# QihanW/eals_cpp

Measured on NVIDIA B200. Metric: eals_nnzK_updates_per_s, higher is better.
Workload: dtype f64

## Files before the change

### eals_cpp_b200/csrc/cd_block.cuh

```cuda
#pragma once

#include "cd_sweep.cuh"
#include "common.cuh"

namespace eals {

constexpr int kBlkThreads = 256;
constexpr int kBlkWarps = kBlkThreads / 32;
constexpr int kPartLen = 208;
constexpr int kMaxSlab = 256;

__device__ __forceinline__ uint32_t tile_chunk_off(int r, int c) { return (uint32_t)(r * 128 + (((c ^ r) & 7) << 4)); }
__device__ __forceinline__ double tile_elem(const unsigned char* tile, int r, int e) {
  return *reinterpret_cast<const double*>(tile + tile_chunk_off(r, e >> 1) + ((e & 1) << 3));
}

__device__ __forceinline__ void cp_async16(void* smem_dst, const void* gmem_src, int src_bytes) {
  const uint32_t d = (uint32_t)__cvta_generic_to_shared(smem_dst);
  asm volatile("cp.async.cg.shared.global [%0], [%1], 16, %2;\n" ::"r"(d), "l"(gmem_src), "r"(src_bytes) : "memory");
}
__device__ __forceinline__ void cp_async_commit() { asm volatile("cp.async.commit_group;\n" ::: "memory"); }
template <int N>
__device__ __forceinline__ void cp_async_wait() { asm volatile("cp.async.wait_group %0;\n" ::"n"(N) : "memory"); }

__device__ __forceinline__ void stage_tile_rows(unsigned char* tile, const double* const* rowp_s, int n, int n_pad,
                                                int fb, int tid, int nthreads) {
  const int c = tid & 7;
  const uint32_t col_bytes = (uint32_t)(fb * (kFB * 8) + c * 16);
  for (int r = tid >> 3; r < n_pad; r += nthreads >> 3) {
    const bool live = r < n;
    const unsigned char* src = reinterpret_cast<const unsigned char*>(rowp_s[live ? r : 0]) + col_bytes;
    cp_async16(tile + (uint32_t)(r * 128) + (uint32_t)(((c ^ r) & 7) << 4), src, live ? 16 : 0);
  }
}

__device__ __forceinline__ void stage_two_tiles(unsigned char* tile_prev, unsigned char* tile, const double* const* rowp_s,
                                                int n, int n_pad, int fb, bool do_prev, bool do_cur, int tid, int nthreads) {
  const int c = tid & 7;
  const uint32_t col_bytes = (uint32_t)(fb * (kFB * 8) + c * 16);
  for (int r = tid >> 3; r < n_pad; r += nthreads >> 3) {
    const bool live = r < n;
    const unsigned char* src = reinterpret_cast<const unsigned char*>(rowp_s[live ? r : 0]) + col_bytes;
    const uint32_t dst = (uint32_t)(r * 128) + (uint32_t)(((c ^ r) & 7) << 4);
    if (do_prev) cp_async16(tile_prev + dst, src - kFB * 8, live ? 16 : 0);
    if (do_cur) cp_async16(tile + dst, src, live ? 16 : 0);
  }
}

__device__ __forceinline__ void dmma_884(double& c0, double& c1, double a, double b) {
  asm volatile("mma.sync.aligned.m8n8k4.row.col.f64.f64.f64.f64 {%0,%1}, {%2}, {%3}, {%0,%1};\n"
               : "+d"(c0), "+d"(c1)
               : "d"(a), "d"(b));
}

__device__ __forceinline__ void load_tile_row(const unsigned char* tile, int r, double (&y)[16]) {
#pragma unroll
  for (int c = 0; c < 8; c++) {
    const double2 d = *reinterpret_cast<const double2*>(tile + tile_chunk_off(r, c));
    y[2 * c] = d.x;
    y[2 * c + 1] = d.y;
  }
}

constexpr int kSBlk = 16 * 17;
constexpr int kGsStride = 17;
constexpr int kGsLen = 16 * kGsStride;
__host__ __device__ constexpr int s_tri(int bi, int bj) { return bi * (bi + 1) / 2 + bj; }

template <int LD, int MAXM>
struct WarpBlockSmem {
  static constexpr bool kSInSmem = LD <= 128;
  static constexpr int kNB = LD / 16;
  static constexpr int kRows = 32 * MAXM;
  static constexpr size_t kS = kSInSmem ? (size_t)s_tri(kNB, 0) * kSBlk * 8 : 0;
  static constexpr size_t kTile = (size_t)kRows * 128;
  static constexpr size_t kBytesPerWarp = kTile + (size_t)kRows * 8 + (size_t)LD * 8 + (kGsLen + 16 + 16) * 8;
  static constexpr int kMaxWarps = MAXM == 1 ? 16 : (MAXM == 2 ? 12 : (MAXM == 3 ? 9 : 7));
};

__device__ __forceinline__ void gram_rhs_fragments(const unsigned char* tile, const double* c_s, const double* z_s,
                                                   int r0, int r1, double (&frag)[10]) {
  const int lane = lane_id();
  const int rr = lane & 3, e0 = lane >> 2;
  const uint32_t off_lo = (uint32_t)(rr * 128 + ((e0 & 1) << 3));
  for (int j0 = r0; j0 < r1; j0 += 4) {
    const int r = j0 + rr;
    const uint32_t sw = (uint32_t)(r & 7);
    const unsigned char* rowp = tile + (size_t)j0 * 128 + off_lo;
    const double a0 = *reinterpret_cast<const double*>(rowp + ((((uint32_t)(e0 >> 1)) ^ sw) << 4));
    const double a1 = *reinterpret_cast<const double*>(rowp + ((((uint32_t)(4 + (e0 >> 1))) ^ sw) << 4));
    const double cj = c_s[r];
    const double zj = e0 == 0 ? z_s[r] : 0.0;
    const double b0 = cj * a0, b1 = cj * a1;
    dmma_884(frag[0], frag[1], a0, b0);
    dmma_884(frag[2], frag[3], a1, b0);
    dmma_884(frag[4], frag[5], a1, b1);
    dmma_884(frag[6], frag[7], a0, zj);
    dmma_884(frag[8], frag[9], a1, zj);
  }
}

__device__ __forceinline__ void gram_rhs_fragments_reg(const unsigned char* tile, double c_lane, double z_lane,
                                                       int r0, int r1, double (&frag)[10]) {
  const int lane = lane_id();
  const int rr = lane & 3, e0 = lane >> 2;
  const uint32_t off_lo = (uint32_t)(rr * 128 + ((e0 & 1) << 3));
  for (int j0 = r0; j0 < r1; j0 += 4) {
    const int r = j0 + rr;
    const uint32_t sw = (uint32_t)(r & 7);
    const unsigned char* rowp = tile + (size_t)j0 * 128 + off_lo;
    const double a0 = *reinterpret_cast<const double*>(rowp + ((((uint32_t)(e0 >> 1)) ^ sw) << 4));
    const double a1 = *reinterpret_cast<const double*>(rowp + ((((uint32_t)(4 + (e0 >> 1))) ^ sw) << 4));
    const double cj = __shfl_sync(kFullMask, c_lane, (j0 - r0) + rr);
    const double zq = __shfl_sync(kFullMask, z_lane, (j0 - r0) + rr);
    const double zj = e0 == 0 ? zq : 0.0;
    const double b0 = cj * a0, b1 = cj * a1;
    dmma_884(frag[0], frag[1], a0, b0);
    dmma_884(frag[2], frag[3], a1, b0);
    dmma_884(frag[4], frag[5], a1, b1);
    dmma_884(frag[6], frag[7], a0, zj);
    dmma_884(frag[8], frag[9], a1, zj);
  }
}

template <int LD, int MAXM, bool USER>
__global__ void __launch_bounds__(WarpBlockSmem<LD, MAXM>::kMaxWarps * 32, 1)
cd_warp_block_kernel(CdSide a, const int32_t* __restrict__ order, int first, int count) {
  extern __shared__ __align__(128) unsigned char smem[];
  using Sm = WarpBlockSmem<LD, MAXM>;
  const int warp = threadIdx.x >> 5, lane = lane_id();
// ... 213 lines not shown
      const double hff = Gs[f * kGsStride + f];
      const double xf = x_s[f0 + f];
      double numer = Pt[f] - g * tsum + xf * hff;
      const double rden = 1.0 / (hff + a.reg);
#pragma unroll
      for (int s = 0; s < 16; s++) {
        const double d = numer * rden - xf;
        const double ds = __shfl_sync(kFullMask, d, s);
        if (f > s) numer -= ds * h[s];
      }
      const double xnew = numer * rden;
      if (lane < 16) {
        const bool livef = f0 + f < K;
        if (livef) x_s[f0 + f] = xnew;
        delta_s[f] = livef ? xnew - xf : 0.0;
      }
      __syncwarp();

      double d[16];
#pragma unroll
      for (int e = 0; e < 16; e++) d[e] = delta_s[e];
#pragma unroll
      for (int m = 0; m < MAXM; m++) {
        const int j = m * 32 + lane;
        if (j < n) {
          double y[16];
          load_tile_row(tile, j, y);
          double a0 = pr[m], a1 = 0.0, a2 = 0.0, a3 = 0.0;
#pragma unroll
          for (int e = 0; e < 16; e += 4) {
            a0 += d[e] * y[e];
            a1 += d[e + 1] * y[e + 1];
            a2 += d[e + 2] * y[e + 2];
            a3 += d[e + 3] * y[e + 3];
          }
          pr[m] = (a0 + a1) + (a2 + a3);
        }
      }
      __syncwarp();
      if (fb + 1 < nblocks) {
        stage_tile_rows(tile, rowp_s, n, n_pad, fb + 1, lane, 32);
        cp_async_commit();
      }
    }
    for (int k = lane; k < K; k += 32) store_row_value(a, (size_t)grow * LD + k, x_s[k]);
    if (a.pc_out.n) {
#pragma unroll
      for (int m = 0; m < MAXM; m++) {
        const int j = m * 32 + lane;
        if (j < n) pc_emit(a, p0 + j, gpos[m], pr[m]);
      }
    }
    for (int st = stages_in_loop; st < 4; st++) fetch_next(st, slot + stride);
    __syncwarp();
  }
  peers_release(a);
}

template <int LD, int TW, int MW>
struct RowBlockSmem {
  static constexpr int kT = TW * 32;
  static constexpr int kRows = kT * MW;
  static constexpr size_t kTile = (size_t)kRows * 128;
  static constexpr size_t kIdx = (size_t)kRows * 8;
  static constexpr size_t kCZ = (size_t)kRows * 16;
  static constexpr size_t kX = (size_t)LD * 8;
  static constexpr size_t kSlots = (size_t)TW * kPartLen * 8;
  static constexpr size_t kSmall = (kGsLen + 16 + 16 + 16 + 16 * 16) * 8;
  static constexpr size_t kBytes = kTile + kIdx + kCZ + kX + kSlots + kSmall;
};

template <int LD, int TW, int MW, bool USER>
__global__ void __launch_bounds__(TW * 32, 16 / TW)
cd_row_block_kernel(CdSide a, const int32_t* __restrict__ order, int first) {
  extern __shared__ __align__(128) unsigned char smem[];
  using Sm = RowBlockSmem<LD, TW, MW>;
  constexpr int kT = TW * 32;
  constexpr int kParts = kT / 16;
  static_assert(kPartLen + 16 <= kT || TW < 8, "reduction threads");
  unsigned char* tile = smem;
  const double** rowp_s = reinterpret_cast<const double**>(smem + Sm::kTile);
  double* c_s = reinterpret_cast<double*>(smem + Sm::kTile + Sm::kIdx);
  double* z_s = c_s + Sm::kRows;
  double* x_s = z_s + Sm::kRows;
  double* slots = x_s + LD;
  double* Gs = slots + TW * kPartLen;
  double* Pt = Gs + kGsLen;
  double* Tt = Pt + 16;
  double* delta_s = Tt + 16;
  double* tpart = delta_s + 16;

  const int tid = threadIdx.x, lane = lane_id(), warp = tid >> 5;
  const int row = order[first + blockIdx.x];
  const int64_t p0 = a.ptr[row];
  const int n = (int)(a.ptr[row + 1] - p0);
  const int n_pad = (n + 3) & ~3;
  const int grow = a.row_base + row;
  double* xrow = a.X + (size_t)grow * LD;
  const int K = a.K;
  const double wi_row = USER ? 0.0 : a.Wi[grow];
  const double g = USER ? 1.0 : wi_row;

  double pr[MW], cw[MW], wr[MW];
#pragma unroll
  for (int m = 0; m < MW; m++) {
    const int j = m * kT + tid;
// ... 429 lines not shown
```

### eals_cpp_b200/csrc/eals_b200.cu

```cuda

#include "../../include/eals_b200.h"

#include <algorithm>
#include <chrono>
#include <cmath>
#include <cstdarg>
#include <cstring>
#include <limits>
#include <new>
#include <random>
#include <string>
#include <thread>
#include <utility>
#include <vector>

#include <cuda.h>
#include <cuda_fp16.h>

#include <cub/device/device_radix_sort.cuh>
#include <cub/device/device_run_length_encode.cuh>
#include <cub/device/device_scan.cuh>
#include <cub/device/device_select.cuh>
#include <thrust/iterator/counting_iterator.h>

// ... 47 lines not shown

template <typename F>
void parallel_chunks(int64_t n, int* n_threads_out, F fn, int64_t min_per_thread = 65536) {
  unsigned hw = std::thread::hardware_concurrency();
  int T = (int)std::min<int64_t>(std::max(1u, std::min(hw, 16u)), std::max<int64_t>(1, n / min_per_thread));
  if (n_threads_out) *n_threads_out = T;
  if (T <= 1) { fn(0, (int64_t)0, n); return; }
  std::vector<std::thread> th;
  const int64_t per = (n + T - 1) / T;
  for (int t = 0; t < T; t++) th.emplace_back(fn, t, std::min(n, t * per), std::min(n, (t + 1) * per));
  for (auto& x : th) x.join();
}
constexpr int kMaxHostThreads = 16;

template <typename T>
int dev_alloc(T** p, size_t n) {
  *p = nullptr;
  if (n == 0) n = 1;
  CU(cudaMalloc((void**)p, n * sizeof(T)));
  return EALS_OK;
}

template <typename T>
int dev_reserve(T** p, size_t* cap, size_t n) {
  if (n == 0) n = 1;
  if (*p && n <= *cap) return EALS_OK;
  cudaFree(*p);
  *p = nullptr;
  *cap = 0;
  CU(cudaMalloc((void**)p, n * sizeof(T)));
  *cap = n;
  return EALS_OK;
}

inline size_t recv_offset(int64_t n) { return ((size_t)n + 15) & ~(size_t)15; }

constexpr int kNumBuckets = 9;
constexpr int kBucketMax[kNumBuckets] = {0, 32, 64, 96, 128, 256, 384, 512, 0x7fffffff};
constexpr int kMidBucket = 5;
constexpr int kHeavyBucket = 8;
constexpr int64_t kDefaultBatchNnz = 4LL * 1024 * 1024 * 1024;

struct HeavyBatch { int h0, h1, u0, u1; };

struct Side {
  int rows = 0;
  int row_base = 0;
  int64_t nnz = 0;
  int64_t* ptr = nullptr;
  int32_t* idx = nullptr;
  double* val = nullptr;
  int32_t* order = nullptr;
  int first[kNumBuckets + 1] = {0};
  int n_hrows = 0, n_units = 0, max_batch_units = 0;
  int64_t heavy_nnz = 0;
  eals::UnitDesc* units_canon = nullptr;
  eals::UnitDesc* units_launch = nullptr;
  int slab = eals::kMaxSlab;
  int32_t *hrow_id = nullptr, *hrow_unit0 = nullptr, *hrow_units = nullptr;
  int32_t *hrow_grp0 = nullptr, *hrow_grps = nullptr, *grp_unit0 = nullptr, *grp_cnt = nullptr;
  int64_t* hrow_poff = nullptr;
  size_t cap_hrow_poff = 0;
  int32_t* unit_launch = nullptr;
  uint32_t *sort_keys = nullptr, *sort_keys_out = nullptr;
  int32_t* sort_vals = nullptr;
  unsigned char* sort_tmp = nullptr;
  size_t cap_sort_keys = 0, cap_sort_keys_out = 0, cap_sort_vals = 0, cap_sort_tmp = 0;
  int n_groups = 0;
  std::vector<int32_t> h_hrow_grp0, h_hrow_grps;
  std::vector<int32_t> h_hrow_unit0, h_hrow_units;
  std::vector<int32_t> h_row_to_hrow;
  std::vector<HeavyBatch> batches;
  double* pred = nullptr;
  double* delta = nullptr;
  size_t cap_ptr = 0, cap_idx = 0, cap_val = 0, cap_order = 0, cap_units_canon = 0, cap_units_launch = 0, cap_hrow_id = 0, cap_hrow_unit0 = 0, cap_hrow_units = 0, cap_pred = 0,
         cap_delta = 0, cap_hrow_grp0 = 0, cap_hrow_grps = 0, cap_grp_unit0 = 0, cap_grp_cnt = 0, cap_unit_launch = 0;
  std::vector<int64_t> h_ptr;
};

enum { T_USER_SWEEP, T_USER_GRAM, T_ITEM_SWEEP, T_ITEM_GRAM, T_LOSS, T_EVAL,
       T_U_HEAVY, T_U_MID, T_U_WARP, T_I_HEAVY, T_I_MID, T_I_WARP, T_COUNT };
constexpr int kPublicTimers = 6;

struct BlockTiming { long long users = 0, items = 0; double ms = 0; };
struct EvalStats { int engine = 0; long long candidates = 0, pairs = 0; BlockTiming blk0; };
struct RecStats { int engine = 0; long long seed = 0, pairs = 0, left1 = 0; BlockTiming blk0; };

}

struct eals_model {
  eals_params p;
  cudaStream_t own_stream = nullptr;
  int K = 0, LD = 0;
  int M = 0, N = 0;
  int ub = 0, ue = 0, ib = 0, ie = 0;
  cudaStream_t stream = nullptr;
  double *U = nullptr, *V = nullptr, *SU = nullptr, *SV = nullptr, *Wi = nullptr;
  double* terms = nullptr;
  double* partials = nullptr;
  size_t partials_len = 0;
  Side users, items;
  int sm_count = 148;
  int64_t launches = 0;
  double last_ms[T_COUNT] = {0};
  std::vector<std::pair<cudaEvent_t, cudaEvent_t>> pending[T_COUNT];
  std::vector<cudaEvent_t> pool;
  double acc_ms[T_COUNT] = {0};
  int64_t acc_calls[T_COUNT] = {0};
  bool factors_set = false;
  struct eals_eval_ws* eval = nullptr;
  EvalStats eval_stats;
  RecStats rec_stats;
  double init_stream_s = 0;
  bool su_fresh = true;
  double* S_tmp = nullptr;
  int* flags = nullptr;
  eals::PeerSet peersU = {}, peersV = {};
  double* pc_u = nullptr;
  double* pc_i = nullptr;
  uint32_t* map_u = nullptr;
  uint32_t* map_i = nullptr;
  size_t cap_pc_u = 0, cap_pc_i = 0, cap_map_u = 0, cap_map_i = 0;
  double *pc_stage_u = nullptr, *pc_stage_i = nullptr;
  uint32_t *route_src_u = nullptr, *route_dst_u = nullptr, *route_src_i = nullptr, *route_dst_i = nullptr;
  size_t cap_stage_u = 0, cap_stage_i = 0, cap_rsrc_u = 0, cap_rdst_u = 0, cap_rsrc_i = 0, cap_rdst_i = 0;
  bool routed = false;
  long long pair_cnt[8][8] = {{0}};
  uint32_t *recv_idx_u = nullptr, *recv_idx_i = nullptr;
  size_t cap_recv_idx_u = 0, cap_recv_idx_i = 0;
  bool copy_route = false;
  bool unpack_u_pending = false, unpack_i_pending = false;
  std::vector<void*> graveyard;
  int ipc_gen = 0;
  int64_t *full_rp = nullptr, *full_cp = nullptr;
  int32_t *full_ci = nullptr, *full_ri = nullptr;
  unsigned char* route_tmp = nullptr;
  size_t cap_full_rp = 0, cap_full_cp = 0, cap_full_ci = 0, cap_full_ri = 0, cap_route_tmp = 0;
  eals::PcOut out_to_items = {}, out_to_users = {};
  int n_ranks = 1, rank = 0;
  cudaStream_t side_stream = nullptr;
  cudaEvent_t ev_swept = nullptr, ev_routed = nullptr;
  cudaStream_t copy_stream[2] = {nullptr, nullptr};
  cudaEvent_t ev_copied[2] = {nullptr, nullptr};
  bool route_pending = false;
  cudaGraphExec_t epoch_graph = nullptr;
  long long graph_key = -1, config_gen = 0;
  long long graph_launches_per_epoch = 0;
  bool capturing = false;
  int route_todo = 0;
  bool local_peers = false;
  bool pc_attached = false;
  bool pc_users_attached = false, pc_items_attached = false;
  bool pcache_on = false;
  bool pc_u_valid = false, pc_i_valid = false;
  int sweeps_since_fresh = 0;
  int pred_refresh_every = 0;
};

namespace {

using eals::CdSide;

int sync_if_debug(eals_model* m) {
  if (m->p.flags & EALS_FLAG_SYNC_EACH_CALL) {
    CU(cudaStreamSynchronize(m->stream));
    CU(cudaGetLastError());
  }
  return EALS_OK;
}

int check_launch(eals_model* m) {
  m->launches++;
  CU(cudaGetLastError());
  return EALS_OK;
}

void free_side(Side& s) {
  cudaFree(s.ptr); cudaFree(s.idx); cudaFree(s.val); cudaFree(s.order);
  cudaFree(s.pred); cudaFree(s.delta);
  cudaFree(s.units_canon); cudaFree(s.units_launch);
  cudaFree(s.hrow_id); cudaFree(s.hrow_unit0); cudaFree(s.hrow_units);
  cudaFree(s.hrow_poff);
  cudaFree(s.hrow_grp0); cudaFree(s.hrow_grps); cudaFree(s.grp_unit0); cudaFree(s.grp_cnt); cudaFree(s.unit_launch);
  cudaFree(s.sort_keys); cudaFree(s.sort_keys_out); cudaFree(s.sort_vals); cudaFree(s.sort_tmp);
  s = Side();
}

template <typename T>
int copy_in(T* dst, const T* src, size_t n, int space, cudaStream_t st) {
  if (n == 0) return EALS_OK;
  CU(cudaMemcpyAsync(dst, src, n * sizeof(T),
                     space == EALS_DEVICE ? cudaMemcpyDeviceToDevice : cudaMemcpyHostToDevice, st));
  return EALS_OK;
}

__global__ void check_indices_kernel(const int32_t* __restrict__ idx, int64_t nnz, int limit,
                                     int* __restrict__ bad, unsigned long long* __restrict__ descents) {
  const int64_t q = (int64_t)blockIdx.x * blockDim.x + threadIdx.x;
  bool oob = false, desc = false;
  if (q < nnz) {
    const int c = idx[q];
    oob = c < 0 || c >= limit;
    desc = q > 0 && idx[q - 1] >= c;
  }
  if (__syncthreads_or(oob) && threadIdx.x == 0) atomicExch(bad, 1);
  const int nd = __syncthreads_count(desc);
  if (nd && threadIdx.x == 0) atomicAdd(descents, (unsigned long long)nd);
}
__global__ void check_row_starts_kernel(const int64_t* __restrict__ ptr, const int32_t* __restrict__ idx, int rows,
                                        unsigned long long* __restrict__ starts) {
  const int r = blockIdx.x * blockDim.x + threadIdx.x;
  bool hit = false;
  if (r < rows) {
    const int64_t q = ptr[r];
    hit = q > 0 && ptr[r + 1] > q && idx[q - 1] >= idx[q];
  }
  const int n = __syncthreads_count(hit);
  if (n && threadIdx.x == 0) atomicAdd(starts, (unsigned long long)n);
}

int ensure_partials(eals_model* m, size_t n);

struct RankBounds {
  int32_t user[9], item[9];
  int n;
};

__global__ void build_maps_kernel(const int64_t* __restrict__ cp, const int32_t* __restrict__ ri, int N,
                                  const int64_t* __restrict__ rp, const int32_t* __restrict__ ci, int64_t nnz,
                                  int ub, int ue, int64_t rp_ub, uint32_t* __restrict__ map_u,
                                  int ib, int ie, int64_t cp_ib, uint32_t* __restrict__ map_i, int* __restrict__ bad,
// ... 357 lines not shown
    sorted_flag = bad;
  }

  tm.lap("side: validate sorted (enqueued)");
  std::vector<int32_t> order((size_t)std::max(s.rows, 1));
  int count[kNumBuckets] = {0};
  constexpr int kLut = kBucketMax[kHeavyBucket - 1] + 2;
  uint8_t lut[kLut];
  for (int n = 0, b = 0; n < kLut; n++) {
    while (n > kBucketMax[b]) b++;
    lut[n] = (uint8_t)b;
  }
  const int heavy_min = getenv("EALS_HEAVY_MIN") ? std::max(32, atoi(getenv("EALS_HEAVY_MIN"))) : kBucketMax[kHeavyBucket - 1];
  for (int n = 0; n < kLut; n++)
    if (n > heavy_min) lut[n] = (uint8_t)kHeavyBucket;
  std::vector<uint8_t> bucket((size_t)std::max(s.rows, 1));
  {
    int T = 1;
    int cnt_t[kMaxHostThreads][kNumBuckets];
    for (auto& c : cnt_t) for (int& v : c) v = 0;
    const int64_t* hp = s.h_ptr.data();
    parallel_chunks(s.rows, &T, [&](int t, int64_t b0, int64_t b1) {
      int local[kNumBuckets] = {0};
      for (int64_t r = b0; r < b1; r++) {
        const int64_t n = hp[r + 1] - hp[r];
        const uint8_t b = lut[std::min<int64_t>(n, kLut - 1)];
        bucket[r] = b;
        local[b]++;
      }
      for (int b = 0; b < kNumBuckets; b++) cnt_t[t][b] = local[b];
    });
    for (int b = 0; b < kNumBuckets; b++)
      for (int t = 0; t < T; t++) count[b] += cnt_t[t][b];
    s.first[0] = 0;
    for (int b = 0; b < kNumBuckets; b++) s.first[b + 1] = s.first[b] + count[b];
    int base_t[kMaxHostThreads][kNumBuckets];
    for (int b = 0; b < kNumBuckets; b++) {
      int at = s.first[b];
      for (int t = 0; t < T; t++) { base_t[t][b] = at; at += cnt_t[t][b]; }
    }
    int T2 = 1;
    parallel_chunks(s.rows, &T2, [&](int t, int64_t b0, int64_t b1) {
      int fill[kNumBuckets];
      for (int b = 0; b < kNumBuckets; b++) fill[b] = base_t[t][b];
      for (int64_t r = b0; r < b1; r++) order[fill[bucket[r]]++] = (int32_t)r;
    });
  }
  std::stable_sort(order.begin() + s.first[kHeavyBucket], order.begin() + s.first[kHeavyBucket + 1],
                   [&](int a, int b) {
                     return s.h_ptr[a + 1] - s.h_ptr[a] > s.h_ptr[b + 1] - s.h_ptr[b];
                   });
  OK(dev_reserve(&s.order, &s.cap_order, order.size()));
  CU(cudaMemcpyAsync(s.order, order.data(), sizeof(int32_t) * order.size(), cudaMemcpyHostToDevice, m->stream));

  if (sorted_flag) {
    int h_flags[6] = {0, 0, 0, 0, 0, 0};
    CU(cudaMemcpyAsync(h_flags, sorted_flag, sizeof(h_flags), cudaMemcpyDeviceToHost, m->stream));
    CU(cudaStreamSynchronize(m->stream));
    unsigned long long h_counts[2];
    std::memcpy(h_counts, h_flags + 2, sizeof(h_counts));
    if (h_flags[0] || h_counts[0] != h_counts[1])
      return fail(EALS_ERR_ARG, "indices inside a row must be strictly ascending and in range");
  }
  tm.lap("side: bucket rows + validate");
  {
    const int hb = s.first[kHeavyBucket], he = s.first[kHeavyBucket + 1];
    s.n_hrows = he - hb;
    std::vector<int32_t> hrow_id, grp_unit0, grp_cnt;
    std::vector<int64_t> hrow_poff;
    int64_t n_units_total = 0;
    s.slab = (getenv("EALS_SLAB") && atoi(getenv("EALS_SLAB")) == 256) ? 256 : 128;
    s.h_hrow_unit0.clear(); s.h_hrow_units.clear(); s.batches.clear(); s.h_row_to_hrow.clear();
    s.h_hrow_grp0.clear(); s.h_hrow_grps.clear();
    {
      int64_t hn = 0;
      for (int h = 0; h < s.n_hrows; h++) { const int r = order[hb + h]; hn += s.h_ptr[r + 1] - s.h_ptr[r]; }
      (void)hn;
      hrow_poff.reserve((size_t)s.n_hrows);
      hrow_id.reserve((size_t)s.n_hrows); s.h_hrow_unit0.reserve((size_t)s.n_hrows); s.h_hrow_units.reserve((size_t)s.n_hrows);
    }
    int64_t poff = 0, batch_nnz = 0;
    int64_t batch_limit = kDefaultBatchNnz;
    if (const char* e = getenv("EALS_HEAVY_BATCH_NNZ")) batch_limit = std::max<int64_t>(atoll(e), 1);
    if (s.n_hrows) s.h_row_to_hrow.assign((size_t)s.rows, -1);
    HeavyBatch cur{0, 0, 0, 0};
    for (int h = 0; h < s.n_hrows; h++) {
      const int r = order[hb + h];
      const int64_t n = s.h_ptr[r + 1] - s.h_ptr[r];
      if (h > cur.h0 && batch_nnz + n > batch_limit) {
        cur.h1 = h; cur.u1 = (int)n_units_total;
        s.batches.push_back(cur);
        cur = HeavyBatch{h, h, cur.u1, cur.u1};
        batch_nnz = 0;
      }
      batch_nnz += n;
      s.h_row_to_hrow[r] = h;
      hrow_id.push_back(r);
      s.h_hrow_unit0.push_back((int)n_units_total);
      hrow_poff.push_back(poff);
      const int nunits = (int)((n + s.slab - 1) / s.slab);
      n_units_total += nunits;
      if (n_units_total >= 0x7fffffffLL) return fail(EALS_ERR_UNSUPPORTED, "too many slabs of heavy rows");
      s.h_hrow_units.push_back(nunits);
      s.h_hrow_grp0.push_back((int)grp_unit0.size());
      s.h_hrow_grps.push_back((nunits + 31) / 32);
      for (int q = 0; q < nunits; q += 32) {
// ... 146 lines not shown
      float f = 0;
      if (pr.second && cudaEventElapsedTime(&f, pr.first, pr.second) == cudaSuccess) {
        m->acc_ms[t] += f;
        m->acc_calls[t]++;
        m->last_ms[t] = f;
      }
      m->pool.push_back(pr.first);
      if (pr.second) m->pool.push_back(pr.second);
    }
    m->pending[t].clear();
  }
}

void tic(eals_model* m, int which) {
  if (m->capturing) return;
  if (m->pending[which].size() >= 2048) { cudaStreamSynchronize(m->stream); fold_timings(m); }
  cudaEvent_t e = take_event(m);
  cudaEventRecord(e, m->stream);
  m->pending[which].emplace_back(e, nullptr);
}
void toc(eals_model* m, int which) {
  if (m->capturing) return;
  cudaEvent_t e = take_event(m);
  cudaEventRecord(e, m->stream);
  m->pending[which].back().second = e;
}

#define DISPATCH_LD(LDV, ...)                                              \
  switch (LDV) {                                                           \
    case 16: { constexpr int LD = 16; __VA_ARGS__; } break;                \
    case 32: { constexpr int LD = 32; __VA_ARGS__; } break;                \
    case 64: { constexpr int LD = 64; __VA_ARGS__; } break;                \
    case 128: { constexpr int LD = 128; __VA_ARGS__; } break;              \
    case 256: { constexpr int LD = 256; __VA_ARGS__; } break;              \
    default: return fail(EALS_ERR_UNSUPPORTED, "leading dimension %d", LDV); \
  }

template <int LD, int MAXM, bool USER>
int launch_cd_warp_block(eals_model* m, const CdSide& a, const int32_t* order, int first, int count) {
  if (count <= 0) return EALS_OK;
  using Sm = eals::WarpBlockSmem<LD, MAXM>;
  const size_t budget = 227 * 1024 - Sm::kS;
  int wpb = (int)std::min<size_t>(Sm::kMaxWarps, std::max<size_t>(1, budget / Sm::kBytesPerWarp));
  static int env_wpb = getenv("EALS_WARP_WPB") ? atoi(getenv("EALS_WARP_WPB")) : 0;
  if (env_wpb > 0) wpb = std::min(env_wpb, wpb);
  const size_t smem = Sm::kS + Sm::kBytesPerWarp * wpb;
  auto kern = eals::cd_warp_block_kernel<LD, MAXM, USER>;
  CU(cudaFuncSetAttribute(kern, cudaFuncAttributeMaxDynamicSharedMemorySize, (int)smem));
  const int grid = std::min((count + wpb - 1) / wpb, m->sm_count);
  kern<<<grid, wpb * 32, smem, m->stream>>>(a, order, first, count);
  return check_launch(m);
}

template <int LD, int TW, int MW, bool USER>
int launch_cd_row_block(eals_model* m, const CdSide& a, const int32_t* order, int first, int count) {
  if (count <= 0) return EALS_OK;
  using Sm = eals::RowBlockSmem<LD, TW, MW>;
  auto kern = eals::cd_row_block_kernel<LD, TW, MW, USER>;
  CU(cudaFuncSetAttribute(kern, cudaFuncAttributeMaxDynamicSharedMemorySize, (int)Sm::kBytes));
  kern<<<count, TW * 32, Sm::kBytes, m->stream>>>(a, order, first);
  return check_launch(m);
}

eals::HeavyUnits heavy_units(const Side& s) {
  eals::HeavyUnits hu;
  hu.units = nullptr;
  hu.hrow_id = s.hrow_id;
  hu.hrow_grp0 = s.hrow_grp0; hu.hrow_grps = s.hrow_grps; hu.grp_unit0 = s.grp_unit0; hu.grp_cnt = s.grp_cnt;
  return hu;
}

template <int LD, bool USER>
int run_heavy_batch(eals_model* m, Side& s, const CdSide& a, const HeavyBatch& b, bool canonical) {
  const int nu = b.u1 - b.u0, nh = b.h1 - b.h0;
  if (nu <= 0) return EALS_OK;
  eals::HeavyUnits hu = heavy_units(s);
  const bool no_order = getenv("EALS_HEAVY_ORDER") && getenv("EALS_HEAVY_ORDER")[0] == '0';
  hu.units = ((canonical && !no_order) ? s.units_launch : s.units_canon) + b.u0;
  const int nblocks = (m->K + eals::kFB - 1) / eals::kFB;
  const int g0 = s.h_hrow_grp0[b.h0];
  const int ngroups = s.h_hrow_grp0[b.h1 - 1] + s.h_hrow_grps[b.h1 - 1] - g0;
  OK(ensure_partials(m, (size_t)(nu + ngroups) * eals::kPartLen));
  double* part = m->partials;
  double* part2 = m->partials + (size_t)nu * eals::kPartLen;
  auto step = s.slab == 256 ? eals::heavy_step_kernel<LD, USER, 256> : eals::heavy_step_kernel<LD, USER, 128>;
  const int step_smem = (int)(s.slab == 256 ? eals::HeavySmem<256>::kBytes : eals::HeavySmem<128>::kBytes);
  CU(cudaFuncSetAttribute(step, cudaFuncAttributeMaxDynamicSharedMemorySize, step_smem));
  if (!a.use_cache) {
    eals::heavy_pred_kernel<LD><<<nu, eals::kBlkThreads, 0, m->stream>>>(a, hu, s.pred);
    OK(check_launch(m));
  }
  for (int fb = 0; fb <= nblocks; fb++) {
    if (fb == nblocks && !a.pc_out.n) break;
    step<<<nu, s.slab, step_smem, m->stream>>>(a, hu, b.u0, fb, nblocks, s.pred, s.delta, part);
    OK(check_launch(m));
    if (fb == nblocks) break;
    eals::heavy_reduce_kernel<<<ngroups, eals::kBlkThreads, 0, m->stream>>>(part, hu, g0, b.u0, part2);
    OK(check_launch(m));
    eals::heavy_solve_kernel<LD, USER><<<nh, eals::kBlkThreads, 0, m->stream>>>(a, hu, b.h0, g0, fb, part2, s.delta);
    OK(check_launch(m));
  }
  return EALS_OK;
}

template <int LD, bool USER>
int launch_cd(eals_model* m, Side& s, const CdSide& a, int only_row) {
  if (only_row >= 0) {
    const int64_t n = s.h_ptr[only_row + 1] - s.h_ptr[only_row];
    if (n == 0) return EALS_OK;
    if (!s.h_row_to_hrow.empty() && s.h_row_to_hrow[only_row] >= 0) {
      const int h = s.h_row_to_hrow[only_row];
      return run_heavy_batch<LD, USER>(m, s, a, HeavyBatch{h, h + 1, s.h_hrow_unit0[h], s.h_hrow_unit0[h] + s.h_hrow_units[h]}, false);
    }
    OK(ensure_partials(m, 16));
    int32_t* one = reinterpret_cast<int32_t*>(m->partials);
    CU(cudaMemcpyAsync(one, &only_row, sizeof(int32_t), cudaMemcpyHostToDevice, m->stream));
    if (n <= 32) return launch_cd_warp_block<LD, 1, USER>(m, a, one, 0, 1);
    if (n <= 64) return launch_cd_warp_block<LD, 2, USER>(m, a, one, 0, 1);
    if (n <= 96) return launch_cd_warp_block<LD, 3, USER>(m, a, one, 0, 1);
    if (n <= 128) return launch_cd_warp_block<LD, 4, USER>(m, a, one, 0, 1);
    if (n <= 256) return launch_cd_row_block<LD, 4, 2, USER>(m, a, one, 0, 1);
    if (n <= 384) return launch_cd_row_block<LD, 4, 3, USER>(m, a, one, 0, 1);
    return launch_cd_row_block<LD, 8, 2, USER>(m, a, one, 0, 1);
  }
  const int t0 = USER ? T_U_HEAVY : T_I_HEAVY;
  tic(m, t0);
  for (const HeavyBatch& b : s.batches) OK((run_heavy_batch<LD, USER>(m, s, a, b, true)));
  toc(m, t0);
  tic(m, t0 + 1);
  OK((launch_cd_row_block<LD, 8, 2, USER>(m, a, s.order, s.first[7], s.first[8] - s.first[7])));
  OK((launch_cd_row_block<LD, 4, 3, USER>(m, a, s.order, s.first[6], s.first[7] - s.first[6])));
  OK((launch_cd_row_block<LD, 4, 2, USER>(m, a, s.order, s.first[5], s.first[6] - s.first[5])));
  toc(m, t0 + 1);
  tic(m, t0 + 2);
  OK((launch_cd_warp_block<LD, 4, USER>(m, a, s.order, s.first[4], s.first[5] - s.first[4])));
  OK((launch_cd_warp_block<LD, 3, USER>(m, a, s.order, s.first[3], s.first[4] - s.first[3])));
  OK((launch_cd_warp_block<LD, 2, USER>(m, a, s.order, s.first[2], s.first[3] - s.first[2])));
  OK((launch_cd_warp_block<LD, 1, USER>(m, a, s.order, s.first[1], s.first[2] - s.first[1])));
  toc(m, t0 + 2);
  return EALS_OK;
}

int launch_route(eals_model* m, bool on_side_stream) {
  if (!m->route_todo) return EALS_OK;
  const bool user = m->route_todo == 1;
  m->route_todo = 0;
  static const bool inline_route = getenv("EALS_ROUTE_INLINE") && getenv("EALS_ROUTE_INLINE")[0] == '1';
  const Side& s = user ? m->users : m->items;
  const eals::PcOut& out = user ? m->out_to_items : m->out_to_users;
  cudaStream_t rs = m->stream;
  if (on_side_stream && !inline_route) {
    CU(cudaStreamWaitEvent(m->side_stream, m->ev_swept, 0));
    rs = m->side_stream;
  }
  if (m->copy_route) {
    const int me = m->rank, nr = m->n_ranks;
    const double* stage = user ? m->pc_stage_u : m->pc_stage_i;
    cudaStream_t lanes[3] = {rs, rs, rs};
    static const bool no_fan = getenv("EALS_COPY_FAN") && getenv("EALS_COPY_FAN")[0] == '0';
    const bool fan = rs != m->stream && nr > 2 && !no_fan;
    if (fan) {
      for (int c = 0; c < 2; c++) {
        if (!m->copy_stream[c]) {
          CU(cudaStreamCreateWithFlags(&m->copy_stream[c], cudaStreamNonBlocking));
          CU(cudaEventCreateWithFlags(&m->ev_copied[c], cudaEventDisableTiming));
        }
        CU(cudaStreamWaitEvent(m->copy_stream[c], m->ev_swept, 0));
        lanes[c + 1] = m->copy_stream[c];
      }
    }
    int n_copy = 0;
    long long seg = 0;
    for (int r = 0; r < nr; r++) {
      const long long cnt = user ? m->pair_cnt[me][r] : m->pair_cnt[r][me];
      long long off = 0;
      for (int q = 0; q < me; q++) off += user ? m->pair_cnt[q][r] : m->pair_cnt[r][q];
      const long long dst_n = (long long)out.bound[r + 1] - (long long)out.bound[r];
      if (cnt > 0 && r != me)
        CU(cudaMemcpyAsync(out.base[r] + recv_offset(dst_n) + off, stage + seg, sizeof(double) * (size_t)cnt, cudaMemcpyDefault,
                           lanes[n_copy++ % 3]));
      seg += cnt;
    }
    if (fan)
      for (int c = 0; c < 2; c++) {
        CU(cudaEventRecord(m->ev_copied[c], m->copy_stream[c]));
        CU(cudaStreamWaitEvent(m->side_stream, m->ev_copied[c], 0));
      }
    if (seg != s.nnz) return fail(EALS_ERR_STATE, "routing table does not cover the staged predictions (%lld of %lld)", seg, (long long)s.nnz);
    (user ? m->unpack_i_pending : m->unpack_u_pending) = true;
  } else {
    const int grid = (int)std::min<int64_t>((s.nnz + 255) / 256, 4 * m->sm_count);
// ... 978 lines not shown
```

Baseline: 275.1 billion.

## Batch several short rows per warp in a new warp-rows CD kernel

Replaces the one-row-per-warp kernel for rows with at most 32 nonzeros with a kernel that packs up to 8 short rows (up to 104 padded lines) into one warp. Rows share a staged Y tile and the S*x tensor-core products, with per-row Gram fragments and a per-row triangular solve. Batch boundaries are computed on the host at setup and uploaded. The aim is to fill warp lanes and MMA fragments that sat mostly idle on short rows, at the cost of more complex indexing, extra shuffles and higher per-warp shared memory.

```diff
diff --git a/eals_cpp_b200/csrc/cd_block.cuh b/eals_cpp_b200/csrc/cd_block.cuh
--- a/eals_cpp_b200/csrc/cd_block.cuh
+++ b/eals_cpp_b200/csrc/cd_block.cuh
@@ -47,6 +47,17 @@
   }
 }
 
+__device__ __forceinline__ void stage_tile_lines(unsigned char* tile, const double* const* rowp_s, const double* any,
+                                                 int nlines, int fb, int lane) {
+  const int c = lane & 7;
+  const uint32_t col_bytes = (uint32_t)(fb * (kFB * 8) + c * 16);
+  for (int r = lane >> 3; r < nlines; r += 4) {
+    const double* p = rowp_s[r];
+    const unsigned char* src = reinterpret_cast<const unsigned char*>(p ? p : any) + col_bytes;
+    cp_async16(tile + (uint32_t)(r * 128) + (uint32_t)(((c ^ r) & 7) << 4), src, p ? 16 : 0);
+  }
+}
+
 __device__ __forceinline__ void dmma_884(double& c0, double& c1, double a, double b) {
   asm volatile("mma.sync.aligned.m8n8k4.row.col.f64.f64.f64.f64 {%0,%1}, {%2}, {%3}, {%0,%1};\n"
                : "+d"(c0), "+d"(c1)
@@ -75,7 +86,7 @@
   static constexpr size_t kS = kSInSmem ? (size_t)s_tri(kNB, 0) * kSBlk * 8 : 0;
   static constexpr size_t kTile = (size_t)kRows * 128;
   static constexpr size_t kBytesPerWarp = kTile + (size_t)kRows * 8 + (size_t)LD * 8 + (kGsLen + 16 + 16) * 8;
-  static constexpr int kMaxWarps = MAXM == 1 ? 16 : (MAXM == 2 ? 12 : (MAXM == 3 ? 9 : 7));
+  static constexpr int kMaxWarps = MAXM == 2 ? 12 : (MAXM == 3 ? 9 : 7);
 };
 
 __device__ __forceinline__ void gram_rhs_fragments(const unsigned char* tile, const double* c_s, const double* z_s,
@@ -395,6 +406,374 @@
       }
     }
     for (int st = stages_in_loop; st < 4; st++) fetch_next(st, slot + stride);
+    __syncwarp();
+  }
+  peers_release(a);
+}
+
+#ifndef EALS_BR
+#define EALS_BR 8
+#define EALS_BL 104
+#endif
+constexpr int kBatchRows = EALS_BR;
+constexpr int kBatchLines = EALS_BL;
+constexpr int kBatchMaxLen = 32;
+
+__host__ __device__ constexpr int swz16(int r) { return (r & 1) | ((r & 2) << 2); }
+__device__ __forceinline__ int kperm(int q, int c) { return 2 * c + (q & 1) + 8 * (q >> 1); }
+constexpr int kHRow = 3 * 64 + 2;
+
+template <int LD>
+struct WarpRowsSmem {
+  static constexpr bool kSInSmem = LD <= 128;
+  static constexpr int kNB = LD / 16;
+  static constexpr int kL = kBatchLines;
+  static constexpr size_t kS = kSInSmem ? (size_t)s_tri(kNB, 0) * 256 * 8 : 0;
+  static constexpr size_t kTile = (size_t)kL * 128;
+  static constexpr int kXStride = LD + 16;
+  static constexpr int kXLen = kBatchRows * kXStride;
+  static constexpr size_t kRaw = kTile + (size_t)kL * 24 + (size_t)kXLen * 8 + (size_t)kBatchRows * kHRow * 8 +
+                                 (size_t)kBatchRows * 18 * 8;
+  static constexpr size_t kBytesPerWarp = (kRaw + 127) & ~(size_t)127;
+  static constexpr int kMaxWarps = 8;
+};
+
+template <int LD, bool USER>
+__global__ void __launch_bounds__(WarpRowsSmem<LD>::kMaxWarps * 32, 1)
+cd_warp_rows_kernel(CdSide a, const int32_t* __restrict__ order, int first, const int32_t* __restrict__ bstart,
+                    int nbatch) {
+  extern __shared__ __align__(128) unsigned char smem[];
+  using Sm = WarpRowsSmem<LD>;
+  constexpr int kL = Sm::kL;
+  constexpr int LM = (kL + 31) / 32;
+  const int warp = threadIdx.x >> 5, lane = lane_id();
+  const int wpb = blockDim.x >> 5;
+
+  const double* S_s = reinterpret_cast<const double*>(smem);
+  if (Sm::kSInSmem) {
+    double* S_w = reinterpret_cast<double*>(smem);
+    for (int t = threadIdx.x; t < s_tri(Sm::kNB, 0) * 256; t += blockDim.x) {
+      const int blk = t >> 8, r = (t >> 4) & 15, c = t & 15;
+      int bi = 0;
+      while (s_tri(bi + 1, 0) <= blk) bi++;
+      const int bj = blk - s_tri(bi, 0);
+      S_w[blk * 256 + r * 16 + (c ^ swz16(r))] = __ldg(a.S + (size_t)(bi * 16 + r) * LD + bj * 16 + c);
+    }
+    __syncthreads();
+  }
+
+  unsigned char* base = smem + Sm::kS + (size_t)warp * Sm::kBytesPerWarp;
+  unsigned char* tile = base;
+  const double** rowp_s = reinterpret_cast<const double**>(base + Sm::kTile);
+  double* c_s = reinterpret_cast<double*>(base + Sm::kTile + (size_t)kL * 8);
+  double* z_s = c_s + kL;
+  double* x_s = z_s + kL;
+  double* H_s = x_s + Sm::kXLen;
+  double* delta_s = H_s + kBatchRows * kHRow;
+
+  const int K = a.K;
+  const int nblocks = (K + kFB - 1) / kFB;
+  const int gr = lane >> 2, gc = lane & 3;
+  const int stride = gridDim.x * wpb;
+
+  int nr_n = 0, row_n = 0, n_n = 0, s_n = 0;
+  int64_t p0_n = 0;
+  double wi_row_n = 0.0;
+  int id_n[LM], rl_n[LM];
+  int64_t k_n[LM];
+  double pc_n[LM], wi_n[LM];
+  uint32_t g_n[LM];
+  bool live_n[LM];
+#pragma unroll
+  for (int m = 0; m < LM; m++) { id_n[m] = 0; rl_n[m] = 0; k_n[m] = 0; pc_n[m] = 0.0; wi_n[m] = 0.0; g_n[m] = 0; live_n[m] = false; }
+  auto fetch_next = [&](int stage, int b) {
+    if (b >= nbatch) return;
+    if (stage == 0) {
+      const int b0 = bstart[b];
+      nr_n = bstart[b + 1] - b0;
+      if (lane < nr_n) row_n = order[first + b0 + lane];
+    } else if (stage == 1) {
+      if (lane < nr_n) {
+        p0_n = a.ptr[row_n];
+        n_n = (int)(a.ptr[row_n + 1] - p0_n);
+        if (!USER) wi_row_n = a.Wi[a.row_base + row_n];
+      }
+    } else if (stage == 2) {
+      const int np = lane < nr_n ? (n_n + 3) & ~3 : 0;
+      int incl = np;
+#pragma unroll
+      for (int o = 1; o < kBatchRows; o <<= 1) {
+        const int v = __shfl_up_sync(kFullMask, incl, o);
+        if (lane >= o) incl += v;
+      }
+      s_n = incl - np;
+#pragma unroll
+      for (int m = 0; m < LM; m++) {
+        const int j = m * 32 + lane;
+        int rl = 0;
+#pragma unroll
+        for (int r = 1; r < kBatchRows; r++) {
+          const int sr = __shfl_sync(kFullMask, s_n, r);
+          if (r < nr_n && j >= sr) rl = r;
+        }
+        const int sr = __shfl_sync(kFullMask, s_n, rl);
+        const int nrl = __shfl_sync(kFullMask, n_n, rl);
+        const int64_t prl = __shfl_sync(kFullMask, p0_n, rl);
+        rl_n[m] = rl;
+        live_n[m] = j - sr < nrl && j < kL;
+        if (live_n[m]) {
+          k_n[m] = prl + (j - sr);
+          id_n[m] = a.idx[k_n[m]];
+          if (a.use_cache) pc_n[m] = a.pc_in[k_n[m]];
+          if (a.pc_out.n) g_n[m] = a.pc_map[k_n[m]];
+        }
+      }
+    } else if (USER) {
+#pragma unroll
+      for (int m = 0; m < LM; m++)
+        if (live_n[m]) wi_n[m] = a.Wi[id_n[m]];
+    }
+  };
+  {
+    const int b0 = blockIdx.x * wpb + warp;
+#pragma unroll
+    for (int st = 0; st < 4; st++) fetch_next(st, b0);
+  }
+
+  for (int b = blockIdx.x * wpb + warp; b < nbatch; b += stride) {
+    const int nr = nr_n;
+    const int row = row_n, n_row = n_n, seg = s_n;
+    const double g_row = USER ? 1.0 : wi_row_n;
+    const int nlines = __shfl_sync(kFullMask, seg + ((n_row + 3) & ~3), nr - 1);
+    const double g_lane = USER ? 1.0 : __shfl_sync(kFullMask, g_row, gr);
+
+    double pr[LM], cw[LM], wr[LM];
+    uint32_t gpos[LM];
+    int64_t kpos[LM];
+    int rl[LM];
+    bool live[LM];
+#pragma unroll
+    for (int m = 0; m < LM; m++) {
+      const int j = m * 32 + lane;
+      live[m] = live_n[m]; rl[m] = rl_n[m]; kpos[m] = k_n[m]; gpos[m] = g_n[m];
+      pr[m] = 0.0; cw[m] = 0.0; wr[m] = 0.0;
+      const double wi_l = USER ? wi_n[m] : __shfl_sync(kFullMask, g_row, rl[m]);
+      if (live[m]) {
+        rowp_s[j] = a.Y + (size_t)id_n[m] * LD;
+        const double w = a.val ? a.val[kpos[m]] : 1.0;
+        wr[m] = w * w;
+        cw[m] = w - wi_l;
+        if (a.use_cache) pr[m] = pc_n[m];
+      } else if (j < kL) {
+        rowp_s[j] = nullptr;
+      }
+      if (j < kL) c_s[j] = cw[m];
+    }
+    for (int r = 0; r < kBatchRows; r++) {
+      const int rowr = __shfl_sync(kFullMask, row, r);
+      const double* xr = a.X + (size_t)(a.row_base + rowr) * LD;
+      double* xs = x_s + r * Sm::kXStride + swz16(r);
+#pragma unroll 4
+      for (int k = lane; k < LD; k += 32) {
+        if (r < nr) xs[k] = xr[k];
+        else xs[k] = 0.0;
+      }
+    }
+    __syncwarp();
+
+    int segr[kBatchRows + 1];
+#pragma unroll
+    for (int r = 0; r < kBatchRows; r++) {
+      const int v = __shfl_sync(kFullMask, seg, r);
+      segr[r] = r < nr ? v : nlines;
+    }
+    segr[kBatchRows] = nlines;
+
+    if (!a.use_cache) {
+      double* ptmp = reinterpret_cast<double*>(tile);
+      const int g8 = lane >> 3, gl = lane & 7;
+      for (int j0 = 0; j0 < nlines; j0 += 4) {
+        const int j = j0 + g8;
+        const double* yrow = rowp_s[j];
+        double acc0 = 0.0, acc1 = 0.0;
+        if (yrow) {
+          int r = 0;
+#pragma unroll
+          for (int q = 1; q < kBatchRows; q++)
+            if (j >= segr[q]) r = q;
+          const double* xr = x_s + r * Sm::kXStride + swz16(r);
+#pragma unroll
+          for (int c = 0; c < LD; c += kFB) {
+            const double2 d = ldg2(yrow + c + gl * 2);
+            acc0 += xr[c + gl * 2] * d.x;
+            acc1 += xr[c + gl * 2 + 1] * d.y;
+          }
+        }
+        double acc = acc0 + acc1;
+        acc += __shfl_xor_sync(kFullMask, acc, 1);
+        acc += __shfl_xor_sync(kFullMask, acc, 2);
+        acc += __shfl_xor_sync(kFullMask, acc, 4);
+        if (yrow && gl == 0) ptmp[j] = acc;
+      }
+      __syncwarp();
+#pragma unroll
+      for (int m = 0; m < LM; m++)
+        if (live[m]) pr[m] = ptmp[m * 32 + lane];
+      __syncwarp();
+    }
+
+    stage_tile_lines(tile, rowp_s, a.Y, nlines, 0, lane);
+    cp_async_commit();
+    const int gx = gr < kBatchRows ? gr : 0;
+    const double* xg = x_s + gx * Sm::kXStride + swz16(gx);
+    const double* Hg = H_s + gx * kHRow;
+    const int hsw = gc & 1;
+    for (int fb = 0; fb < nblocks; fb++) {
+      const int f0 = fb * kFB;
+      if (fb < 4) fetch_next(fb, b + stride);
+      auto sx_block = [&](int kb, double (&acc)[4]) {
+#pragma unroll
+        for (int q = 0; q < 4; q++) {
+          const int kk = kperm(q, gc);
+          const double av = xg[kb * 16 + kk];
+          double b0, b1;
+          if (Sm::kSInSmem) {
+            if (kb >= fb) {
+              const double* blk = S_s + s_tri(kb, fb) * 256 + kk * 16;
+              b0 = blk[gr ^ swz16(kk)];
+              b1 = blk[(gr + 8) ^ swz16(kk)];
+            } else {
+              const double* blk = S_s + s_tri(fb, kb) * 256 + (kk ^ swz16(gr));
+              b0 = blk[gr * 16];
+              b1 = blk[(gr + 8) * 16];
+            }
+          } else {
+            const double* sc = a.S + (size_t)(kb * 16 + kk) * LD + f0 + gr;
+            b0 = __ldg(sc);
+            b1 = __ldg(sc + 8);
+          }
+          dmma_884(acc[0], acc[1], av, b0);
+          dmma_884(acc[2], acc[3], av, b1);
+        }
+      };
+      double t[4] = {0.0, 0.0, 0.0, 0.0}, u[4] = {0.0, 0.0, 0.0, 0.0};
+      for (int kb = 0; kb < Sm::kNB; kb += 2) {
+        sx_block(kb, t);
+        if (kb + 1 < Sm::kNB) sx_block(kb + 1, u);
+      }
+#pragma unroll
+      for (int i = 0; i < 4; i++) t[i] += u[i];
+      double sbb[6];
+#pragma unroll
+      for (int tt = 0; tt < 3; tt++) {
+#pragma unroll
+        for (int ii = 0; ii < 2; ii++) {
+          const int rw = gr + (tt >= 1 ? 8 : 0), cl = 2 * gc + ii + (tt == 2 ? 8 : 0);
+          sbb[2 * tt + ii] = Sm::kSInSmem ? S_s[s_tri(fb, fb) * 256 + rw * 16 + (cl ^ swz16(rw))]
+                                          : __ldg(a.S + (size_t)(f0 + rw) * LD + f0 + cl);
+        }
+      }
+      cp_async_wait<0>();
+#pragma unroll
+      for (int m = 0; m < LM; m++) {
+        const int j = m * 32 + lane;
+        if (j < kL) z_s[j] = wr[m] - cw[m] * pr[m];
+      }
+      __syncwarp();
+
+      double pv[4] = {0.0, 0.0, 0.0, 0.0};
+#pragma unroll
+      for (int r = 0; r < kBatchRows; r++) {
+        if (r >= nr) break;
+        double frag[10] = {0, 0, 0, 0, 0, 0, 0, 0, 0, 0};
+        gram_rhs_fragments(tile, c_s, z_s, segr[r], segr[r + 1], frag);
+        const double g = USER ? 1.0 : __shfl_sync(kFullMask, g_row, r);
+        double* Hr = H_s + r * kHRow;
+#pragma unroll
+        for (int tt = 0; tt < 3; tt++) {
+#pragma unroll
+          for (int ii = 0; ii < 2; ii++) {
+            const int cl = 2 * gc + ii;
+            Hr[tt * 64 + gr * 8 + (cl ^ ((gr >> 1) & 1))] = frag[2 * tt + ii] + g * sbb[2 * tt + ii];
+          }
+        }
+#pragma unroll
+        for (int i = 0; i < 4; i++) {
+          const double v = __shfl_sync(kFullMask, (i >> 1) ? frag[8] : frag[6], (kperm(i, gc) & 7) * 4);
+          if (gr == r) pv[i] = v;
+        }
+      }
+      __syncwarp();
+
+      double xf[4], numer[4], rden[4];
+#pragma unroll
+      for (int i = 0; i < 4; i++) {
+        const int f = kperm(i, gc), rr = f & 7;
+        const double hff = Hg[(i >> 1) * 128 + rr * 8 + (rr ^ hsw)];
+        xf[i] = xg[f0 + f];
+        numer[i] = pv[i] - g_lane * t[i] + xf[i] * hff;
+        rden[i] = 1.0 / (hff + a.reg);
+      }
+#pragma unroll
+      for (int s = 0; s < 16; s++) {
+        const int is = (s & 1) + 2 * (s >> 3);
+        const double d = numer[is] * rden[is] - xf[is];
+        const double ds = __shfl_sync(kFullMask, d, (lane & ~3) | ((s & 7) >> 1));
+#pragma unroll
+        for (int i = 0; i < 4; i++) {
+          if (i < 2 && s >= 8) continue;
+          const int f = kperm(i, gc);
+          const int tt = i < 2 ? 0 : (s < 8 ? 1 : 2);
+          if (f > s) numer[i] -= ds * Hg[tt * 64 + (f & 7) * 8 + ((s & 7) ^ hsw)];
+        }
+      }
+      if (gr < nr) {
+#pragma unroll
+        for (int i = 0; i < 4; i++) {
+          const int f = kperm(i, gc);
+          const double xnew = numer[i] * rden[i];
+          const bool livef = f0 + f < K;
+          if (livef) x_s[gr * Sm::kXStride + swz16(gr) + f0 + f] = xnew;
+          delta_s[gr * 18 + f] = livef ? xnew - xf[i] : 0.0;
+        }
+      }
+      __syncwarp();
+
+#pragma unroll
+      for (int m = 0; m < LM; m++) {
+        if (live[m]) {
+          double y[16];
+          load_tile_row(tile, m * 32 + lane, y);
+          const double* d = delta_s + rl[m] * 18;
+          double a0 = pr[m], a1 = 0.0, a2 = 0.0, a3 = 0.0;
+#pragma unroll
+          for (int e = 0; e < 16; e += 4) {
+            a0 += d[e] * y[e];
+            a1 += d[e + 1] * y[e + 1];
+            a2 += d[e + 2] * y[e + 2];
+            a3 += d[e + 3] * y[e + 3];
+          }
+          pr[m] = (a0 + a1) + (a2 + a3);
+        }
+      }
+      __syncwarp();
+      if (fb + 1 < nblocks) {
+        stage_tile_lines(tile, rowp_s, a.Y, nlines, fb + 1, lane);
+        cp_async_commit();
+      }
+    }
+    for (int r = 0; r < nr; r++) {
+      const int rowr = __shfl_sync(kFullMask, row, r);
+      const double* xs = x_s + r * Sm::kXStride + swz16(r);
+      const size_t off = (size_t)(a.row_base + rowr) * LD;
+      for (int k = lane; k < K; k += 32) store_row_value(a, off + k, xs[k]);
+    }
+    if (a.pc_out.n) {
+#pragma unroll
+      for (int m = 0; m < LM; m++)
+        if (live[m]) pc_emit(a, kpos[m], gpos[m], pr[m]);
+    }
+    for (int st = nblocks < 4 ? nblocks : 4; st < 4; st++) fetch_next(st, b + stride);
     __syncwarp();
   }
   peers_release(a);
diff --git a/eals_cpp_b200/csrc/eals_b200.cu b/eals_cpp_b200/csrc/eals_b200.cu
--- a/eals_cpp_b200/csrc/eals_b200.cu
+++ b/eals_cpp_b200/csrc/eals_b200.cu
@@ -123,6 +123,8 @@
   double* val = nullptr;
   int32_t* order = nullptr;
   int first[kNumBuckets + 1] = {0};
+  int32_t* batch = nullptr;
+  int n_batches = 0;
   int n_hrows = 0, n_units = 0, max_batch_units = 0;
   int64_t heavy_nnz = 0;
   eals::UnitDesc* units_canon = nullptr;
@@ -144,6 +146,7 @@
   std::vector<HeavyBatch> batches;
   double* pred = nullptr;
   double* delta = nullptr;
+  size_t cap_batch = 0;
   size_t cap_ptr = 0, cap_idx = 0, cap_val = 0, cap_order = 0, cap_units_canon = 0, cap_units_launch = 0, cap_hrow_id = 0, cap_hrow_unit0 = 0, cap_hrow_units = 0, cap_pred = 0,
          cap_delta = 0, cap_hrow_grp0 = 0, cap_hrow_grps = 0, cap_grp_unit0 = 0, cap_grp_cnt = 0, cap_unit_launch = 0;
   std::vector<int64_t> h_ptr;
@@ -247,7 +250,7 @@
 }
 
 void free_side(Side& s) {
-  cudaFree(s.ptr); cudaFree(s.idx); cudaFree(s.val); cudaFree(s.order);
+  cudaFree(s.ptr); cudaFree(s.idx); cudaFree(s.val); cudaFree(s.order); cudaFree(s.batch);
   cudaFree(s.pred); cudaFree(s.delta);
   cudaFree(s.units_canon); cudaFree(s.units_launch);
   cudaFree(s.hrow_id); cudaFree(s.hrow_unit0); cudaFree(s.hrow_units);
@@ -711,6 +714,21 @@
                    });
   OK(dev_reserve(&s.order, &s.cap_order, order.size()));
   CU(cudaMemcpyAsync(s.order, order.data(), sizeof(int32_t) * order.size(), cudaMemcpyHostToDevice, m->stream));
+  static_assert(kBucketMax[1] == eals::kBatchMaxLen && eals::kBatchMaxLen <= eals::kBatchLines, "short-row batches");
+  std::vector<int32_t> batch(1, 0);
+  for (int i = s.first[1], rows = 0, lines = 0; i < s.first[2]; i++) {
+    const int pad = (int)((s.h_ptr[order[i] + 1] - s.h_ptr[order[i]] + 3) & ~3);
+    if (rows == eals::kBatchRows || lines + pad > eals::kBatchLines) {
+      batch.push_back(i - s.first[1]);
+      rows = lines = 0;
+    }
+    rows++;
+    lines += pad;
+  }
+  if (s.first[2] > s.first[1]) batch.push_back(s.first[2] - s.first[1]);
+  s.n_batches = (int)batch.size() - 1;
+  OK(dev_reserve(&s.batch, &s.cap_batch, batch.size()));
+  CU(cudaMemcpyAsync(s.batch, batch.data(), sizeof(int32_t) * batch.size(), cudaMemcpyHostToDevice, m->stream));
 
   if (sorted_flag) {
     int h_flags[6] = {0, 0, 0, 0, 0, 0};
@@ -963,6 +981,20 @@
   return check_launch(m);
 }
 
+template <int LD, bool USER>
+int launch_cd_warp_rows(eals_model* m, const CdSide& a, const int32_t* order, int first, const int32_t* batch, int n_batches) {
+  if (n_batches <= 0) return EALS_OK;
+  using Sm = eals::WarpRowsSmem<LD>;
+  const size_t budget = 227 * 1024 - Sm::kS;
+  const int wpb = (int)std::min<size_t>(Sm::kMaxWarps, std::max<size_t>(1, budget / Sm::kBytesPerWarp));
+  const size_t smem = Sm::kS + Sm::kBytesPerWarp * wpb;
+  auto kern = eals::cd_warp_rows_kernel<LD, USER>;
+  CU(cudaFuncSetAttribute(kern, cudaFuncAttributeMaxDynamicSharedMemorySize, (int)smem));
+  const int grid = std::min((n_batches + wpb - 1) / wpb, m->sm_count);
+  kern<<<grid, wpb * 32, smem, m->stream>>>(a, order, first, batch, n_batches);
+  return check_launch(m);
+}
+
 template <int LD, int TW, int MW, bool USER>
 int launch_cd_row_block(eals_model* m, const CdSide& a, const int32_t* order, int first, int count) {
   if (count <= 0) return EALS_OK;
@@ -1025,8 +1057,9 @@
     }
     OK(ensure_partials(m, 16));
     int32_t* one = reinterpret_cast<int32_t*>(m->partials);
-    CU(cudaMemcpyAsync(one, &only_row, sizeof(int32_t), cudaMemcpyHostToDevice, m->stream));
-    if (n <= 32) return launch_cd_warp_block<LD, 1, USER>(m, a, one, 0, 1);
+    const int32_t h_one[3] = {only_row, 0, 1};
+    CU(cudaMemcpyAsync(one, h_one, sizeof(h_one), cudaMemcpyHostToDevice, m->stream));
+    if (n <= 32) return launch_cd_warp_rows<LD, USER>(m, a, one, 0, one + 1, 1);
     if (n <= 64) return launch_cd_warp_block<LD, 2, USER>(m, a, one, 0, 1);
     if (n <= 96) return launch_cd_warp_block<LD, 3, USER>(m, a, one, 0, 1);
     if (n <= 128) return launch_cd_warp_block<LD, 4, USER>(m, a, one, 0, 1);
@@ -1047,7 +1080,7 @@
   OK((launch_cd_warp_block<LD, 4, USER>(m, a, s.order, s.first[4], s.first[5] - s.first[4])));
   OK((launch_cd_warp_block<LD, 3, USER>(m, a, s.order, s.first[3], s.first[4] - s.first[3])));
   OK((launch_cd_warp_block<LD, 2, USER>(m, a, s.order, s.first[2], s.first[3] - s.first[2])));
-  OK((launch_cd_warp_block<LD, 1, USER>(m, a, s.order, s.first[1], s.first[2] - s.first[1])));
+  OK((launch_cd_warp_rows<LD, USER>(m, a, s.order, s.first[1], s.batch, s.n_batches)));
   toc(m, t0 + 2);
   return EALS_OK;
 }
```

Result: slower. 267.6 billion, median of 6 (-2.7%).
